# vituslcx/Shuffle-exchange

Hardware: AMD Instinct MI355X
Metric: tokens/sec Llama-3-8B ZeRO-3 bf16 (training, whole job) (higher is better)
Workload: dtype bf16; 1 GPU; llama8b-z3; model=llama3-8b, global_batch=16, seq_len=2048, micro_batch_per_gpu=8, grad_accum=2, parallelism=zero3-dp1, params=8030261248, activation_checkpointing=False, optimizer=AdamW(fp32 master, fused HIP), zero_knobs=tuned, sequence_parallel_size=1, expert_parallel_size=1

## Files before the change

csrc/kernels/gemm_wgrad.hip:

```cpp
#include "sxe_common.h"
#include <torch/library.h>

namespace sxe {
namespace wg {

constexpr int BM = 256, BN = 256, SLAB = 16;
constexpr int NWAVE = 8, NTHR = NWAVE * 64;
constexpr int ROWB = 256;
constexpr int HALF = SLAB * ROWB;
constexpr int SLOT = 4 * HALF;
constexpr int GROUP_M = 8;

typedef __bf16 bf16x8 __attribute__((ext_vector_type(8)));
typedef short i16x4 __attribute__((ext_vector_type(4)));
typedef short i16x8 __attribute__((ext_vector_type(8)));
typedef float f32x16 __attribute__((ext_vector_type(16)));

__device__ __forceinline__ int swz(int row) { return (row & 3) << 2; }

__device__ __forceinline__ i16x4 lds_tr(const char* base, int byte_off) {
  return __builtin_amdgcn_ds_read_tr16_b64_v4i16(
      (__attribute__((address_space(3))) i16x4*)(const_cast<char*>(base) + byte_off));
}

__device__ __forceinline__ int frag_off(int dt, int lane) {
  const int g = lane >> 4, i = lane & 15, q = i >> 2, p = i & 3, h = g >> 1;
  const int ch = 4 * dt + 2 * (g & 1) + (p >> 1);
  const int row = 4 * h + q;
  return row * ROWB + 16 * (ch ^ swz(row)) + 8 * (p & 1);
}

__device__ __forceinline__ bf16x8 frag_at(const char* lane_base, int row0) {
  i16x4 lo = lds_tr(lane_base, row0 * ROWB);
  i16x4 hi = lds_tr(lane_base, (row0 + 8) * ROWB);
  const i16x8 c = __builtin_shufflevector(lo, hi, 0, 1, 2, 3, 4, 5, 6, 7);
  return __builtin_bit_cast(bf16x8, c);
}

__device__ __forceinline__ void glds16(const void* gsrc, unsigned lds) {
  asm volatile("s_mov_b32 m0, %0\n\tglobal_load_lds_dwordx4 %1, off" ::"s"(lds), "v"(gsrc) : "memory", "m0");
}

struct DmaPlan {
  const unsigned short* a;
  const unsigned short* b;
  unsigned lds_a, lds_b;
};

__device__ __forceinline__ DmaPlan dma_plan(const unsigned short* A, int64_t lda, const unsigned short* B,
                                            int64_t ldb, int m0, int n0, unsigned lds_base) {
  const int lane = threadIdx.x & 63, w = threadIdx.x >> 6;
  const int half = (w >> 2) & 1, rq = w & 3;
  const int row = 4 * rq + (lane >> 4);
  const int ch = (lane & 15) ^ swz(row);
  DmaPlan d;
  d.a = A + (int64_t)row * lda + m0 + half * 128 + ch * 8;
  d.b = B + (int64_t)row * ldb + n0 + half * 128 + ch * 8;
  d.lds_a = __builtin_amdgcn_readfirstlane(lds_base + half * HALF + 4 * rq * ROWB);
  d.lds_b = __builtin_amdgcn_readfirstlane(lds_base + (2 + half) * HALF + 4 * rq * ROWB);
  return d;
}

__device__ __forceinline__ void load_slab(const DmaPlan& d, int64_t lda, int64_t ldb, int slab, int slot) {
  const int r = SLAB * slab;
  glds16(d.a + (int64_t)r * lda, d.lds_a + slot * SLOT);
  glds16(d.b + (int64_t)r * ldb, d.lds_b + slot * SLOT);
}

__device__ __forceinline__ int acc_row(int i, int h) { return (i & 3) + 8 * (i >> 2) + 4 * h; }

template <bool ACCUM, int R, bool STAGGER, bool NODMA = false, bool SEG2 = false>
__global__ void __launch_bounds__(NTHR, 1) wgrad_kernel(const unsigned short* __restrict__ A, int64_t lda,
                                                        const unsigned short* __restrict__ B, int64_t ldb,
                                                        float* __restrict__ C, int64_t ldc, int M, int N, int K,
                                                        float alpha, int group_m, const unsigned short* A2,
                                                        const unsigned short* B2, int ns1) {
  static_assert(R == 8, "fragment bases assume slots 0-3 / 4-7");
  constexpr int D = STAGGER ? R - 3 : R - 2;
  constexpr int WAIT = STAGGER ? 2 * (D - 2) : 2 * (D - 1);
  extern __shared__ __attribute__((aligned(1024))) char smem[];
  const int lane = threadIdx.x & 63, w = threadIdx.x >> 6;
  const int wr = w >> 2, wc = w & 3;
  const int tm = M / BM, tn = N / BN, nwg = tm * tn;
  const int orig = blockIdx.x;
  const int q = nwg / 8, r = nwg % 8, xcd = orig % 8;
  const int wgid = (xcd < r ? xcd * (q + 1) : r * (q + 1) + (xcd - r) * q) + orig / 8;
  const int per_group = group_m * tn;
  const int grp = wgid / per_group;
  const int first_m = grp * group_m;
  const int gsz = min(tm - first_m, group_m);
  const int bm = first_m + (wgid % per_group) % gsz;
  const int bn = (wgid % per_group) / gsz;
  const int m0 = bm * BM, n0 = bn * BN;

  f32x16 acc[4][2];
#pragma unroll
  for (int i = 0; i < 4; ++i)
#pragma unroll
    for (int j = 0; j < 2; ++j)
#pragma unroll
      for (int e = 0; e < 16; ++e) acc[i][j][e] = 0.f;

  const int ns = K / SLAB;
  bf16x8 fa[2][4], fb[2][2];
  const char* fbase[2][6];
#pragma unroll
  for (int h = 0; h < 2; ++h) {
#pragma unroll
    for (int i = 0; i < 4; ++i) fbase[h][i] = smem + 4 * h * SLOT + wr * HALF + frag_off(i, lane);
#pragma unroll
    for (int j = 0; j < 2; ++j)
      fbase[h][4 + j] = smem + 4 * h * SLOT + (2 + (wc >> 1)) * HALF + frag_off((wc & 1) * 2 + j, lane);
  }
  auto read_frags = [&](int slot, bf16x8 (&a)[4], bf16x8 (&b)[2]) {
#pragma unroll
    for (int i = 0; i < 4; ++i) a[i] = frag_at(fbase[slot >> 2][i] + (slot & 3) * SLOT, 0);
#pragma unroll
    for (int j = 0; j < 2; ++j) b[j] = frag_at(fbase[slot >> 2][4 + j] + (slot & 3) * SLOT, 0);
  };
  auto mma = [&](const bf16x8 (&a)[4], const bf16x8 (&b)[2]) {
    __builtin_amdgcn_s_setprio(1);
#pragma unroll
    for (int i = 0; i < 4; ++i)
#pragma unroll
      for (int j = 0; j < 2; ++j) acc[i][j] = __builtin_amdgcn_mfma_f32_32x32x16_bf16(a[i], b[j], acc[i][j], 0, 0, 0);
    __builtin_amdgcn_s_setprio(0);
  };
  const unsigned lds_base = (unsigned)(uintptr_t)(__attribute__((address_space(3))) char*)smem;
  const DmaPlan dp = dma_plan(A, lda, B, ldb, m0, n0, lds_base);
  const DmaPlan dp2 = SEG2 ? dma_plan(A2, lda, B2, ldb, m0, n0, lds_base) : dp;
  auto load_any = [&](int slab, int slot) {
    if (!SEG2 || slab < ns1)
      load_slab(dp, lda, ldb, slab, slot);
    else
      load_slab(dp2, lda, ldb, slab - ns1, slot);
  };
#pragma unroll
  for (int j = 0; j < D; ++j) load_any(j, j);
  asm volatile("s_waitcnt vmcnt(%0)" ::"n"(WAIT) : "memory");
  __builtin_amdgcn_s_barrier();
  read_frags(0, fa[0], fb[0]);
  if (STAGGER && __builtin_amdgcn_readfirstlane(wr) == 1) __builtin_amdgcn_s_barrier();
  for (int s0 = 0; s0 < ns; s0 += R) {
#pragma unroll
    for (int j = 0; j < R; ++j) {
      if (!NODMA) load_any(min(s0 + j + D, ns - 1), (j + D) % R);
      if (NODMA)
        asm volatile("s_waitcnt vmcnt(0)" ::: "memory");
      else
        asm volatile("s_waitcnt vmcnt(%0)" ::"n"(WAIT) : "memory");
      __builtin_amdgcn_s_barrier();
      read_frags((j + 1) % R, fa[(j + 1) & 1], fb[(j + 1) & 1]);
      mma(fa[j & 1], fb[j & 1]);
      if (STAGGER) __builtin_amdgcn_s_barrier();
    }
  }
  if (STAGGER && __builtin_amdgcn_readfirstlane(wr) == 0) __builtin_amdgcn_s_barrier();
  asm volatile("s_waitcnt vmcnt(0)" ::: "memory");
  const int h = lane >> 5, col = lane & 31;
#pragma unroll
  for (int i = 0; i < 4; ++i) {
    float* rowp[2];
    float old[2][16];
#pragma unroll
    for (int j = 0; j < 2; ++j) {
      rowp[j] = C + (int64_t)(m0 + wr * 128 + i * 32) * ldc + n0 + wc * 64 + j * 32 + col;
      if (ACCUM) {
#pragma unroll
        for (int e = 0; e < 16; ++e) old[j][e] = __builtin_nontemporal_load(rowp[j] + (int64_t)acc_row(e, h) * ldc);
      }
    }
#pragma unroll
    for (int j = 0; j < 2; ++j)
#pragma unroll
      for (int e = 0; e < 16; ++e) {
        const float v = alpha * acc[i][j][e];
        rowp[j][(int64_t)acc_row(e, h) * ldc] = ACCUM ? old[j][e] + v : v;
      }
  }
}


namespace w4 {
constexpr int SLAB = 32, R = 4, D = 3;
constexpr int NTHR = 256;
constexpr int HALF = SLAB * ROWB;
constexpr int SLOT = 4 * HALF;
constexpr int WAIT = 8 * (D - 1);

struct Plan {
  const unsigned short* a;
  const unsigned short* b;
  unsigned lds;
};

template <bool ACCUM>
__global__ void __launch_bounds__(NTHR, 1) kernel(const unsigned short* __restrict__ A, int64_t lda,
                                                  const unsigned short* __restrict__ B, int64_t ldb,
                                                  float* __restrict__ C, int64_t ldc, int M, int N, int K,
                                                  float alpha, int group_m, const unsigned short* A2,
                                                  const unsigned short* B2, int ns1) {
  extern __shared__ __attribute__((aligned(1024))) char smem[];
  const int lane = threadIdx.x & 63, w = threadIdx.x >> 6;
  const int wr = w >> 1, wc = w & 1;
  const int tm = M / BM, tn = N / BN, nwg = tm * tn;
  const int orig = blockIdx.x;
  const int q = nwg / 8, r = nwg % 8, xcd = orig % 8;
  const int wgid = (xcd < r ? xcd * (q + 1) : r * (q + 1) + (xcd - r) * q) + orig / 8;
  const int per_group = group_m * tn;
  const int grp = wgid / per_group;
  const int first_m = grp * group_m;
  const int gsz = min(tm - first_m, group_m);
  const int bm = first_m + (wgid % per_group) % gsz;
  const int bn = (wgid % per_group) / gsz;
  const int m0 = bm * BM, n0 = bn * BN;

  f32x16 acc[4][4];
#pragma unroll
  for (int i = 0; i < 4; ++i)
#pragma unroll
    for (int j = 0; j < 4; ++j)
#pragma unroll
      for (int e = 0; e < 16; ++e) acc[i][j][e] = 0.f;

  Plan pl, pl2;
  {
    const int row = lane >> 4;
    const int ch = (lane & 15) ^ swz(row);
    pl.a = A + (int64_t)row * lda + m0 + ch * 8;
    pl.b = B + (int64_t)row * ldb + n0 + ch * 8;
    pl.lds = (unsigned)(uintptr_t)(__attribute__((address_space(3))) char*)smem;
    pl2 = pl;
    pl2.a = A2 + (int64_t)row * lda + m0 + ch * 8;
    pl2.b = B2 + (int64_t)row * ldb + n0 + ch * 8;
  }
  const int ns1_32 = ns1 / 2;
  auto load_slab = [&](int slab_any, int slot) {
    const bool second = slab_any >= ns1_32;
    const Plan& P = second ? pl2 : pl;
    const int slab = second ? slab_any - ns1_32 : slab_any;
#pragma unroll
    for (int it = 0; it < 8; ++it) {
      const int op = it >> 2, half = (it >> 1) & 1, rq = (it & 1) * 4 + w;
      const int64_t rows = (int64_t)SLAB * slab + 4 * rq;
      const unsigned short* src = op == 0 ? P.a + rows * lda + half * 128 : P.b + rows * ldb + half * 128;
      const unsigned dst = __builtin_amdgcn_readfirstlane(pl.lds + slot * SLOT + (op * 2 + half) * HALF + 4 * rq * ROWB);
      glds16(src, dst);
    }
  };
  const char* fa_base[2][4];
  const char* fb_base[2][4];
#pragma unroll
  for (int hb = 0; hb < 2; ++hb)
#pragma unroll
    for (int i = 0; i < 4; ++i) {
      fa_base[hb][i] = smem + 2 * hb * SLOT + wr * HALF + frag_off(i, lane);
      fb_base[hb][i] = smem + 2 * hb * SLOT + (2 + wc) * HALF + frag_off(i, lane);
    }
  bf16x8 fa[2][2][4], fb[2][2][4];
  auto read_frags = [&](int slot, bf16x8 (&a)[2][4], bf16x8 (&b)[2][4]) {
#pragma unroll
    for (int kk = 0; kk < 2; ++kk)
#pragma unroll
      for (int i = 0; i < 4; ++i) {
        a[kk][i] = frag_at(fa_base[slot >> 1][i] + (slot & 1) * SLOT, 16 * kk);
        b[kk][i] = frag_at(fb_base[slot >> 1][i] + (slot & 1) * SLOT, 16 * kk);
      }
  };
  auto mma = [&](const bf16x8 (&a)[2][4], const bf16x8 (&b)[2][4]) {
    __builtin_amdgcn_s_setprio(1);
#pragma unroll
    for (int kk = 0; kk < 2; ++kk)
#pragma unroll
      for (int i = 0; i < 4; ++i)
#pragma unroll
        for (int j = 0; j < 4; ++j)
          acc[i][j] = __builtin_amdgcn_mfma_f32_32x32x16_bf16(a[kk][i], b[kk][j], acc[i][j], 0, 0, 0);
    __builtin_amdgcn_s_setprio(0);
  };
  const int ns = K / SLAB;
#pragma unroll
  for (int j = 0; j < D; ++j) load_slab(j, j);
  asm volatile("s_waitcnt vmcnt(%0)" ::"n"(WAIT) : "memory");
  __builtin_amdgcn_s_barrier();
  read_frags(0, fa[0], fb[0]);
  for (int s0 = 0; s0 < ns; s0 += R) {
#pragma unroll
    for (int j = 0; j < R; ++j) {
      load_slab(min(s0 + j + D, ns - 1), (j + D) % R);
      asm volatile("s_waitcnt vmcnt(%0)\n\ts_waitcnt lgkmcnt(0)" ::"n"(WAIT) : "memory");
      __builtin_amdgcn_s_barrier();
      read_frags((j + 1) % R, fa[(j + 1) & 1], fb[(j + 1) & 1]);
      mma(fa[j & 1], fb[j & 1]);
    }
  }
  asm volatile("s_waitcnt vmcnt(0)" ::: "memory");
  const int h = lane >> 5, col = lane & 31;
#pragma unroll
  for (int i = 0; i < 4; ++i) {
    float* rowp[4];
    float old[4][16];
#pragma unroll
    for (int j = 0; j < 4; ++j) {
      rowp[j] = C + (int64_t)(m0 + wr * 128 + i * 32) * ldc + n0 + wc * 128 + j * 32 + col;
      if (ACCUM) {
#pragma unroll
        for (int e = 0; e < 16; ++e) old[j][e] = __builtin_nontemporal_load(rowp[j] + (int64_t)acc_row(e, h) * ldc);
      }
    }
#pragma unroll
    for (int j = 0; j < 4; ++j)
#pragma unroll
      for (int e = 0; e < 16; ++e) {
        const float v = alpha * acc[i][j][e];
        rowp[j][(int64_t)acc_row(e, h) * ldc] = ACCUM ? old[j][e] + v : v;
      }
  }
}
}

}

bool wgrad_supported(const at::Tensor& a, const at::Tensor& b, const at::Tensor& c) {
  return a.is_cuda() && a.scalar_type() == at::kBFloat16 && b.scalar_type() == at::kBFloat16 &&
         c.scalar_type() == at::kFloat && a.dim() == 2 && b.dim() == 2 && c.dim() == 2 && a.stride(1) == 1 &&
         b.stride(1) == 1 && c.stride(1) == 1 && a.size(0) == b.size(0) && c.size(0) == a.size(1) &&
         c.size(1) == b.size(1) && a.size(1) % wg::BM == 0 && b.size(1) % wg::BN == 0 && a.size(0) % (8 * wg::SLAB) == 0 &&
         (reinterpret_cast<uintptr_t>(a.data_ptr()) % 16 == 0) && (reinterpret_cast<uintptr_t>(b.data_ptr()) % 16 == 0) &&
         a.stride(0) % 8 == 0 && b.stride(0) % 8 == 0;
}

static void wgrad_launch(const at::Tensor& a, const at::Tensor& b, const at::Tensor& a2, const at::Tensor& b2, int K,
                         int ns1, at::Tensor c, double alpha, bool accumulate, int64_t variant, bool seg2 = false) {
  c10::DeviceGuard g(a.device());
  const int M = a.size(1), N = b.size(1);
  const int nwg = (M / wg::BM) * (N / wg::BN);
  const size_t lds = 8 * wg::SLOT;
  using Kern = void (*)(const unsigned short*, int64_t, const unsigned short*, int64_t, float*, int64_t, int, int,
                        int, float, int, const unsigned short*, const unsigned short*, int);
  const int group_m = variant >= 16 ? (int)(variant >> 4) : wg::GROUP_M;
  variant &= 15;
  static const Kern kerns[5][2] = {{wg::wgrad_kernel<false, 8, false>, wg::wgrad_kernel<true, 8, false>},
                                   {wg::wgrad_kernel<false, 8, true>, wg::wgrad_kernel<true, 8, true>},
                                   {wg::w4::kernel<false>, wg::w4::kernel<true>},
                                   {wg::wgrad_kernel<false, 8, false, true>, wg::wgrad_kernel<true, 8, false, true>},
                                   {wg::wgrad_kernel<false, 8, false, false, true>,
                                    wg::wgrad_kernel<true, 8, false, false, true>}};
  static bool attr_set = [&] {
    for (auto& row : kerns)
      for (Kern k : row)
        SXE_HIP_CHECK(hipFuncSetAttribute((const void*)k, hipFuncAttributeMaxDynamicSharedMemorySize, (int)lds));
    return true;
  }();
  (void)attr_set;
  SXE_CHECK(variant >= 0 && variant <= 3, "wgrad_gemm_: variant must be 0..3");
  SXE_CHECK(!seg2 || variant == 0, "wgrad_gemm2_: the 8-wave lock-step schedule only");
  const int nthr = variant == 2 ? wg::w4::NTHR : wg::NTHR;
  hipLaunchKernelGGL(kerns[seg2 ? 4 : variant][accumulate ? 1 : 0], dim3(nwg), dim3(nthr), lds, cur_stream(),
                     reinterpret_cast<const unsigned short*>(a.data_ptr()), a.stride(0),
                     reinterpret_cast<const unsigned short*>(b.data_ptr()), b.stride(0), c.data_ptr<float>(),
                     c.stride(0), M, N, K, (float)alpha, group_m, reinterpret_cast<const unsigned short*>(a2.data_ptr()),
                     reinterpret_cast<const unsigned short*>(b2.data_ptr()), ns1);
  SXE_LAUNCH_CHECK();
}

void wgrad_gemm_variant_(const at::Tensor& a, const at::Tensor& b, at::Tensor c, double alpha, bool accumulate,
                         int64_t variant) {
  SXE_CHECK(wgrad_supported(a, b, c), "wgrad_gemm_: unsupported shapes/dtypes/strides");
  const int K = a.size(0);
  wgrad_launch(a, b, a, b, K, K / wg::SLAB, c, alpha, accumulate, variant);
}

static int64_t default_variant(const at::Tensor& a, const at::Tensor& b) {
  const int64_t tm = a.size(1) / wg::BM, tn = b.size(1) / wg::BN;
  return 0 + 16 * (tm >= 4 * tn ? 4 : 8);
}

void wgrad_gemm_(const at::Tensor& a, const at::Tensor& b, at::Tensor c, double alpha, bool accumulate) {
  wgrad_gemm_variant_(a, b, c, alpha, accumulate, default_variant(a, b));
}

bool wgrad2_supported(const at::Tensor& a, const at::Tensor& b, const at::Tensor& a2, const at::Tensor& b2,
                      const at::Tensor& c) {
  if (a2.dim() != 2 || b2.dim() != 2 || a2.scalar_type() != a.scalar_type() || b2.scalar_type() != b.scalar_type() ||
      a2.size(1) != a.size(1) || b2.size(1) != b.size(1) || a2.size(0) != b2.size(0) || a2.stride(1) != 1 ||
      b2.stride(1) != 1 || a2.stride(0) != a.stride(0) || b2.stride(0) != b.stride(0) || a.size(0) % 32 != 0 ||
      (reinterpret_cast<uintptr_t>(a2.data_ptr()) % 16) != 0 || (reinterpret_cast<uintptr_t>(b2.data_ptr()) % 16) != 0)
    return false;
  const int64_t K = a.size(0) + a2.size(0);
  if (K % (8 * wg::SLAB) != 0) return false;
  return a.is_cuda() && a.scalar_type() == at::kBFloat16 && b.scalar_type() == at::kBFloat16 &&
         c.scalar_type() == at::kFloat && a.dim() == 2 && b.dim() == 2 && c.dim() == 2 && a.stride(1) == 1 &&
         b.stride(1) == 1 && c.stride(1) == 1 && a.size(0) == b.size(0) && c.size(0) == a.size(1) &&
         c.size(1) == b.size(1) && a.size(1) % wg::BM == 0 && b.size(1) % wg::BN == 0 &&
         (reinterpret_cast<uintptr_t>(a.data_ptr()) % 16 == 0) && (reinterpret_cast<uintptr_t>(b.data_ptr()) % 16 == 0) &&
         a.stride(0) % 8 == 0 && b.stride(0) % 8 == 0;
}

void wgrad_gemm2_(const at::Tensor& a, const at::Tensor& b, const at::Tensor& a2, const at::Tensor& b2, at::Tensor c,
                  double alpha, bool accumulate) {
  SXE_CHECK(wgrad2_supported(a, b, a2, b2, c), "wgrad_gemm2_: unsupported shapes/dtypes/strides");
  const int K = (int)(a.size(0) + a2.size(0));
  wgrad_launch(a, b, a2, b2, K, (int)(a.size(0) / wg::SLAB), c, alpha, accumulate, default_variant(a, b), true);
}

}

TORCH_LIBRARY_FRAGMENT(sxe, m) {
  m.def("wgrad_gemm_(Tensor a, Tensor b, Tensor(a!) c, float alpha, bool accumulate) -> ()");
  m.def("wgrad_gemm_variant_(Tensor a, Tensor b, Tensor(a!) c, float alpha, bool accumulate, int variant) -> ()");
  m.def("wgrad_gemm2_(Tensor a, Tensor b, Tensor a2, Tensor b2, Tensor(a!) c, float alpha, bool accumulate) -> ()");
}
TORCH_LIBRARY_IMPL(sxe, CUDA, m) {
  m.impl("wgrad_gemm_", &sxe::wgrad_gemm_);
  m.impl("wgrad_gemm_variant_", &sxe::wgrad_gemm_variant_);
  m.impl("wgrad_gemm2_", &sxe::wgrad_gemm2_);
}
```

shuffle_exchange_amd/ops/linear.py:

```python
import os
import weakref

import torch
import torch.nn.functional as F

TN_MIN_ELEMS = int(os.environ.get("SXE_WGRAD_TN_MIN_ELEMS", 32 * 2**20))
TN_FP32_OUT = os.environ.get("SXE_WGRAD_TN_FP32OUT", "1") == "1"

SKINNY_MAX_M = int(os.environ.get("SXE_SKINNY_MAX_M", 4))


def _skinny(x, weight, bias):
    if torch.compiler.is_compiling():
        return None
    K = x.shape[-1]
    if not (x.is_cuda and x.dtype == torch.bfloat16 and weight.dtype == torch.bfloat16 and weight.dim() == 2
            and weight.is_contiguous() and K % 8 == 0 and weight.data_ptr() % 16 == 0):
        return None
    if bias is not None and not (bias.dtype == torch.bfloat16 and bias.is_contiguous()):
        return None
    x2 = x.reshape(-1, K)
    if not (0 < x2.shape[0] <= SKINNY_MAX_M and x2.stride(1) == 1 and x2.stride(0) % 8 == 0
            and x2.data_ptr() % 16 == 0):
        return None
    from . import native
    native.require_hip()
    return torch.ops.sxe.skinny_gemm(x2, weight, bias).view(*x.shape[:-1], weight.shape[0])


def _pro_weight(weight):
    if isinstance(weight, torch.Tensor):
        if weight.dtype == torch.bfloat16 and weight.dim() == 2 and weight.is_contiguous() and weight.data_ptr() % 16 == 0:
            return weight, None
        return None
    from .fp_quantizer import FP8Weight
    if not isinstance(weight, FP8Weight):
        return None
    q, sc = weight.q, weight.scale
    if q.element_size() == 1 and q.dim() == 2 and q.is_contiguous():
        return q.view(torch.uint8), sc
    return None


def _pro_ok(x, rows_max=4):
    return (x.is_cuda and x.dtype == torch.bfloat16 and x.dim() == 2 and 0 < x.shape[0] <= rows_max
            and x.stride(1) == 1 and x.stride(0) % 8 == 0 and x.data_ptr() % 16 == 0 and not x.requires_grad)


def fused_rms_linear(x, residual, norm_weight, eps, weight, bias=None):
    wk = _pro_weight(weight)
    if wk is None or not _pro_ok(x) or norm_weight.dtype != torch.bfloat16 or not norm_weight.is_contiguous():
        return None
    if residual is not None and (residual.shape != x.shape or residual.stride() != x.stride()
                                 or residual.dtype != x.dtype):
        return None
    w, sc = wk
    if x.shape[1] != w.shape[1]:
        return None
    y, h = torch.ops.sxe.skinny_gemm_pro(x, residual, norm_weight, float(eps), w, sc, bias, 1)
    return y, (h if residual is not None else x)


def fused_rms_rope_linear(x, residual, norm_weight, eps, weight, rope, positions, cache, slots, nq, nkv):
    wk = _pro_weight(weight)
    if (wk is None or not _pro_ok(x) or norm_weight.dtype != torch.bfloat16 or not norm_weight.is_contiguous()
            or rope.cos.shape[-1] != 64 or not cache.is_contiguous() or cache.dim() != 5 or cache.shape[-1] != 128):
        return None
    if residual is not None and (residual.shape != x.shape or residual.stride() != x.stride()
                                 or residual.dtype != x.dtype):
        return None
    w, sc = wk
    if x.shape[1] != w.shape[1] or w.shape[0] != (nq + 2 * nkv) * 128:
        return None
    y, h = torch.ops.sxe.skinny_gemm_pro_rope(x, residual, norm_weight, float(eps), w, sc, rope.cos, rope.sin,
                                              positions.reshape(-1).contiguous().long(), slots, cache, int(nq), int(nkv))
    return y, (h if residual is not None else x)


def fused_swiglu_linear(gu, weight, bias=None):
    wk = _pro_weight(weight)
    if wk is None or not _pro_ok(gu):
        return None
    w, sc = wk
    if gu.shape[1] != 2 * w.shape[1]:
        return None
    return torch.ops.sxe.skinny_gemm_pro(gu, None, None, 0.0, w, sc, bias, 2)[0]


def fused_merge_linear(part_o, part_ml, weight, bias=None):
    wk = _pro_weight(weight)
    if wk is None or not part_o.is_cuda or part_o.shape[1] > 4:
        return None
    w, sc = wk
    if w.shape[1] != part_o.shape[2] * part_o.shape[3]:
        return None
    return torch.ops.sxe.skinny_gemm_merge(part_o, part_ml, w, sc, bias)


SXE_WGRAD = os.environ.get("SXE_WGRAD", "1") == "1"
WGRAD_MIN_TILES = int(os.environ.get("SXE_WGRAD_MIN_TILES", "768"))


def _sxe_wgrad_ok(gy2, x2, buf):
    if not (SXE_WGRAD and gy2.is_cuda and buf.dtype == torch.float32 and gy2.dtype == torch.bfloat16
            and x2.dtype == torch.bfloat16 and buf.is_contiguous() and gy2.stride(1) == 1 and x2.stride(1) == 1):
        return False
    K, M, N = gy2.shape[0], gy2.shape[1], x2.shape[1]
    if K % 128 or M % 256 or N % 256 or gy2.stride(0) % 8 or x2.stride(0) % 8 or M * N >= 2 ** 27:
        return False
    tiles = (M // 256) * (N // 256)
    return tiles % 256 == 0 or tiles >= WGRAD_MIN_TILES


def _tn_ok(gy2, x2):
    return (gy2.is_cuda and gy2.dtype == torch.bfloat16 and x2.dtype == torch.bfloat16 and TN_MIN_ELEMS > 0
            and gy2.shape[1] * x2.shape[1] >= TN_MIN_ELEMS and gy2.shape[0] % 64 == 0 and gy2.shape[1] % 64 == 0
            and x2.shape[1] % 64 == 0 and gy2.is_contiguous() and x2.is_contiguous())


DGRAD_WT_MIN_ELEMS = int(os.environ.get("SXE_DGRAD_WT_MIN_ELEMS", 16 * 2**20))


WT_CACHE = False
WT_CACHE_MAX_BYTES = int(float(os.environ.get("SXE_WT_CACHE_GB", "20")) * 2**30)
_wt_cache = {}
_wt_cache_bytes = 0


def invalidate_transposed_weights():
    global _wt_cache_bytes
    _wt_cache.clear()
    _wt_cache_bytes = 0


def _transpose16(t):
    return torch.ops.sxe.transpose16(t)


def _transposed_weight(w):
    global _wt_cache_bytes
    if not WT_CACHE or not isinstance(w, torch.nn.Parameter):
        return _transpose16(w)
    hit = _wt_cache.get(id(w))
    if (hit is not None and hit[0]() is w and hit[1].shape == w.shape[::-1] and hit[2] == w.data_ptr()
            and hit[3] == w._version):
        return hit[1]
    if hit is not None:
        _wt_cache.pop(id(w))
        _wt_cache_bytes -= hit[1].numel() * hit[1].element_size()
    wt = _transpose16(w)
    nbytes = wt.numel() * wt.element_size()
    if _wt_cache_bytes + nbytes <= WT_CACHE_MAX_BYTES:
        _wt_cache[id(w)] = (weakref.ref(w), wt, w.data_ptr(), w._version)
        _wt_cache_bytes += nbytes
    return wt


def transposed_weight_cache_bytes():
    return _wt_cache_bytes


def configure_transposed_weight_cache(enabled, free_bytes=None):
    global WT_CACHE, WT_CACHE_MAX_BYTES
    WT_CACHE = bool(enabled)
    cap = int(float(os.environ.get("SXE_WT_CACHE_GB", "20")) * 2**30)
    if free_bytes is not None:
        cap = min(cap, int(free_bytes) // 4)
    WT_CACHE_MAX_BYTES = cap
    invalidate_transposed_weights()
    return cap


def data_grad(gy, w):
    if (DGRAD_WT_MIN_ELEMS > 0 and gy.is_cuda and gy.dtype == torch.bfloat16 and w.dtype == torch.bfloat16
            and w.dim() == 2 and w.is_contiguous() and w.numel() >= DGRAD_WT_MIN_ELEMS and w.shape[0] % 64 == 0
            and w.shape[1] % 64 == 0 and gy.numel() // gy.shape[-1] >= 2048):
        return torch.matmul(gy, _transposed_weight(w).t())
    return torch.matmul(gy, w)


def grad_target(w):
    tgt = getattr(w, "_sxe_grad_target", None)
    if tgt is None or getattr(w, "_sxe_grad_partial", False) or w.grad is not None:
        return None
    return tgt


def write_weight_grad(w, gy2, x2):
    tgt = grad_target(w)
    if tgt is None:
        return False
    buf, accumulate = tgt(w)
    if _sxe_wgrad_ok(gy2, x2, buf):
        torch.ops.sxe.wgrad_gemm_(gy2, x2, buf, 1.0, bool(accumulate))
    elif _tn_ok(gy2, x2) and buf.is_contiguous():
        a, b = torch.ops.sxe.transpose16(gy2), torch.ops.sxe.transpose16(x2).t()
        if buf.dtype == gy2.dtype and not accumulate:
            torch.mm(a, b, out=buf)
        elif buf.dtype == torch.float32 and TN_FP32_OUT:
            torch.ops.aten.addmm.dtype_out(buf, a, b, torch.float32, beta=1 if accumulate else 0, alpha=1, out=buf)
        else:
            dw = torch.mm(a, b).view_as(buf)
            buf.add_(dw) if accumulate else buf.copy_(dw)
    elif buf.dtype == torch.float32 and gy2.dtype != torch.float32:
        if gy2.is_cuda:
            torch.ops.aten.addmm.dtype_out(buf, gy2.t(), x2, torch.float32, beta=1 if accumulate else 0, alpha=1,
                                           out=buf)
        else:
            dw = (gy2.t() @ x2).float()
            buf.add_(dw) if accumulate else buf.copy_(dw)
    elif accumulate:
        buf.addmm_(gy2.t(), x2)
    else:
        torch.mm(gy2.t(), x2, out=buf)
    w._sxe_grad_done(w)
    return True


def _autocast_dtype(x):
    dev = x.device.type
    if dev in ("cuda", "cpu") and torch.is_autocast_enabled(dev):
        return torch.get_autocast_dtype(dev)
    return None


class _Linear(torch.autograd.Function):
    @staticmethod
    def forward(ctx, x, weight, bias):
        ctx.param = None
        ac = _autocast_dtype(x)
        if ac is not None and weight.dtype != ac:
            ctx.param = weight
            x, weight = x.to(ac), weight.to(ac)
            bias = bias.to(ac) if bias is not None else None
        ctx.save_for_backward(x, weight)
        ctx.has_bias = bias is not None
        return F.linear(x, weight, bias)

    @staticmethod
    def backward(ctx, gy):
        x, w = ctx.saved_tensors
        wp = ctx.param if ctx.param is not None else w
        if gy.dtype != x.dtype:
            gy = gy.to(x.dtype)
        gy2 = gy.reshape(-1, gy.shape[-1])
        dx = dw = db = None
        if ctx.needs_input_grad[0]:
            dx = data_grad(gy, w)
        if ctx.needs_input_grad[1]:
            x2 = x.reshape(-1, x.shape[-1])
            if not write_weight_grad(wp, gy2, x2):
                dw = gy2.t() @ x2
        if ctx.has_bias and ctx.needs_input_grad[2]:
            db = gy2.sum(0)
        return dx, dw, db


def linear(x, weight, bias=None):
    if not isinstance(weight, torch.Tensor):
        return weight.linear(x, bias)
    grad = torch.is_grad_enabled() and (weight.requires_grad or x.requires_grad)
    if grad and weight.requires_grad and hasattr(weight, "_sxe_grad_target"):
        return _Linear.apply(x, weight, bias)
    if not grad and SKINNY_MAX_M > 0 and x.is_cuda:
        y = _skinny(x, weight, bias)
        if y is not None:
            return y
    return F.linear(x, weight, bias)


class Linear(torch.nn.Linear):

    _sxe_lower_precision_safe = True

    def __init__(self, in_features, out_features, bias=True, device=None, dtype=None, init_std=None):
        super().__init__(in_features, out_features, bias=bias, device=device, dtype=dtype)
        if init_std is not None:
            with torch.no_grad():
                self.weight.normal_(0.0, init_std)
                if self.bias is not None:
                    self.bias.zero_()
            self._sxe_inited = True

    def forward(self, x, skip_bias=False):
        return linear(x, self.weight, None if skip_bias else self.bias)


class Embedding(torch.nn.Embedding):

    def __init__(self, num_embeddings, embedding_dim, init_std=None, **kw):
        super().__init__(num_embeddings, embedding_dim, **kw)
        if init_std is not None:
            with torch.no_grad():
                self.weight.normal_(0.0, init_std)
            self._sxe_inited = True
```

Measured before the change: 25850 tokens/s.

## Add 4-wave deep-pipelined wgrad GEMM kernel and make it the default

```diff
diff --git a/csrc/kernels/gemm_wgrad.hip b/csrc/kernels/gemm_wgrad.hip
--- a/csrc/kernels/gemm_wgrad.hip
+++ b/csrc/kernels/gemm_wgrad.hip
@@ -1,5 +1,6 @@
 #include "sxe_common.h"
 #include <torch/library.h>
+#include <cstdlib>
 
 namespace sxe {
 namespace wg {
@@ -319,6 +320,125 @@
 }
 }
 
+namespace w4p {
+using w4::HALF;
+using w4::NTHR;
+using w4::SLAB;
+using w4::SLOT;
+constexpr int R = 4, D = 4;
+constexpr int WAIT = 8 * (D - 2);
+
+template <bool ACCUM>
+__global__ void __launch_bounds__(NTHR, 1) kernel(const unsigned short* __restrict__ A, int64_t lda,
+                                                  const unsigned short* __restrict__ B, int64_t ldb,
+                                                  float* __restrict__ C, int64_t ldc, int M, int N, int K,
+                                                  float alpha, int group_m, const unsigned short* A2,
+                                                  const unsigned short* B2, int ns1) {
+  extern __shared__ __attribute__((aligned(1024))) char smem[];
+  const int lane = threadIdx.x & 63, w = threadIdx.x >> 6;
+  const int wr = w >> 1, wc = w & 1;
+  const int tm = M / BM, tn = N / BN, nwg = tm * tn;
+  const int orig = blockIdx.x;
+  const int q = nwg / 8, r = nwg % 8, xcd = orig % 8;
+  const int wgid = (xcd < r ? xcd * (q + 1) : r * (q + 1) + (xcd - r) * q) + orig / 8;
+  const int per_group = group_m * tn;
+  const int grp = wgid / per_group;
+  const int first_m = grp * group_m;
+  const int gsz = min(tm - first_m, group_m);
+  const int bm = first_m + (wgid % per_group) % gsz;
+  const int bn = (wgid % per_group) / gsz;
+  const int m0 = bm * BM, n0 = bn * BN;
+
+  f32x16 acc[4][4];
+#pragma unroll
+  for (int i = 0; i < 4; ++i)
+#pragma unroll
+    for (int j = 0; j < 4; ++j)
+#pragma unroll
+      for (int e = 0; e < 16; ++e) acc[i][j][e] = 0.f;
+
+  const int drow = lane >> 4;
+  const int dch = (lane & 15) ^ swz(drow);
+  const unsigned short* pa = A + (int64_t)drow * lda + m0 + dch * 8;
+  const unsigned short* pb = B + (int64_t)drow * ldb + n0 + dch * 8;
+  const unsigned lds0 = (unsigned)(uintptr_t)(__attribute__((address_space(3))) char*)smem;
+  auto dma = [&](int it, int slab, int slot) {
+    const int op = it >> 2, half = (it >> 1) & 1, rq = (it & 1) * 4 + w;
+    const int64_t rows = (int64_t)SLAB * slab + 4 * rq;
+    const unsigned short* src = op == 0 ? pa + rows * lda + half * 128 : pb + rows * ldb + half * 128;
+    glds16(src, __builtin_amdgcn_readfirstlane(lds0 + slot * SLOT + (op * 2 + half) * HALF + 4 * rq * ROWB));
+  };
+  const char* fa_base[2][4];
+  const char* fb_base[2][4];
+#pragma unroll
+  for (int hb = 0; hb < 2; ++hb)
+#pragma unroll
+    for (int i = 0; i < 4; ++i) {
+      fa_base[hb][i] = smem + 2 * hb * SLOT + wr * HALF + frag_off(i, lane);
+      fb_base[hb][i] = smem + 2 * hb * SLOT + (2 + wc) * HALF + frag_off(i, lane);
+    }
+  bf16x8 fa[2][2][4], fb[2][2][4];
+  auto read_frag = [&](int slot, int f, bf16x8 (&a)[2][4], bf16x8 (&b)[2][4]) {
+    const int kk = f >> 3, i = f & 3;
+    if ((f & 4) == 0)
+      b[kk][i] = frag_at(fb_base[slot >> 1][i] + (slot & 1) * SLOT, 16 * kk);
+    else
+      a[kk][i] = frag_at(fa_base[slot >> 1][i] + (slot & 1) * SLOT, 16 * kk);
+  };
+  const int ns = K / SLAB;
+#pragma unroll
+  for (int j = 0; j < D; ++j)
+#pragma unroll
+    for (int it = 0; it < 8; ++it) dma(it, j, j);
+  asm volatile("s_waitcnt vmcnt(%0)" ::"n"(8 * (D - 1)) : "memory");
+  __builtin_amdgcn_s_barrier();
+#pragma unroll
+  for (int f = 0; f < 16; ++f) read_frag(0, f, fa[0], fb[0]);
+  for (int s0 = 0; s0 < ns; s0 += R) {
+#pragma unroll
+    for (int j = 0; j < R; ++j) {
+      asm volatile("s_waitcnt vmcnt(%0)\n\ts_waitcnt lgkmcnt(0)" ::"n"(WAIT) : "memory");
+      __builtin_amdgcn_s_barrier();
+      __builtin_amdgcn_sched_barrier(0);
+      const int nslab = min(s0 + j + D, ns - 1);
+#pragma unroll
+      for (int g = 0; g < 8; ++g) {
+        const int kk = g >> 2, i = g & 3;
+        dma(g, nslab, j);
+        read_frag((j + 1) % R, 2 * g, fa[(j + 1) & 1], fb[(j + 1) & 1]);
+        read_frag((j + 1) % R, 2 * g + 1, fa[(j + 1) & 1], fb[(j + 1) & 1]);
+#pragma unroll
+        for (int jj = 0; jj < 4; ++jj)
+          acc[i][jj] = __builtin_amdgcn_mfma_f32_32x32x16_bf16(fa[j & 1][kk][i], fb[j & 1][kk][jj], acc[i][jj], 0, 0, 0);
+        __builtin_amdgcn_sched_barrier(0);
+      }
+    }
+  }
+  asm volatile("s_waitcnt vmcnt(0)" ::: "memory");
+  const int h = lane >> 5, col = lane & 31;
+#pragma unroll
+  for (int i = 0; i < 4; ++i) {
+    float* rowp[4];
+    float old[4][16];
+#pragma unroll
+    for (int j = 0; j < 4; ++j) {
+      rowp[j] = C + (int64_t)(m0 + wr * 128 + i * 32) * ldc + n0 + wc * 128 + j * 32 + col;
+      if (ACCUM) {
+#pragma unroll
+        for (int e = 0; e < 16; ++e) old[j][e] = __builtin_nontemporal_load(rowp[j] + (int64_t)acc_row(e, h) * ldc);
+      }
+    }
+#pragma unroll
+    for (int j = 0; j < 4; ++j)
+#pragma unroll
+      for (int e = 0; e < 16; ++e) {
+        const float v = alpha * acc[i][j][e];
+        rowp[j][(int64_t)acc_row(e, h) * ldc] = ACCUM ? old[j][e] + v : v;
+      }
+  }
+}
+}
+
 }
 
 bool wgrad_supported(const at::Tensor& a, const at::Tensor& b, const at::Tensor& c) {
@@ -340,10 +460,11 @@
                         int, float, int, const unsigned short*, const unsigned short*, int);
   const int group_m = variant >= 16 ? (int)(variant >> 4) : wg::GROUP_M;
   variant &= 15;
-  static const Kern kerns[5][2] = {{wg::wgrad_kernel<false, 8, false>, wg::wgrad_kernel<true, 8, false>},
+  static const Kern kerns[6][2] = {{wg::wgrad_kernel<false, 8, false>, wg::wgrad_kernel<true, 8, false>},
                                    {wg::wgrad_kernel<false, 8, true>, wg::wgrad_kernel<true, 8, true>},
                                    {wg::w4::kernel<false>, wg::w4::kernel<true>},
                                    {wg::wgrad_kernel<false, 8, false, true>, wg::wgrad_kernel<true, 8, false, true>},
+                                   {wg::w4p::kernel<false>, wg::w4p::kernel<true>},
                                    {wg::wgrad_kernel<false, 8, false, false, true>,
                                     wg::wgrad_kernel<true, 8, false, false, true>}};
   static bool attr_set = [&] {
@@ -353,10 +474,10 @@
     return true;
   }();
   (void)attr_set;
-  SXE_CHECK(variant >= 0 && variant <= 3, "wgrad_gemm_: variant must be 0..3");
+  SXE_CHECK(variant >= 0 && variant <= 4, "wgrad_gemm_: variant must be 0..4");
   SXE_CHECK(!seg2 || variant == 0, "wgrad_gemm2_: the 8-wave lock-step schedule only");
-  const int nthr = variant == 2 ? wg::w4::NTHR : wg::NTHR;
-  hipLaunchKernelGGL(kerns[seg2 ? 4 : variant][accumulate ? 1 : 0], dim3(nwg), dim3(nthr), lds, cur_stream(),
+  const int nthr = variant == 2 || variant == 4 ? wg::w4::NTHR : wg::NTHR;
+  hipLaunchKernelGGL(kerns[seg2 ? 5 : variant][accumulate ? 1 : 0], dim3(nwg), dim3(nthr), lds, cur_stream(),
                      reinterpret_cast<const unsigned short*>(a.data_ptr()), a.stride(0),
                      reinterpret_cast<const unsigned short*>(b.data_ptr()), b.stride(0), c.data_ptr<float>(),
                      c.stride(0), M, N, K, (float)alpha, group_m, reinterpret_cast<const unsigned short*>(a2.data_ptr()),
@@ -371,9 +492,18 @@
   wgrad_launch(a, b, a, b, K, K / wg::SLAB, c, alpha, accumulate, variant);
 }
 
+static int64_t default_group_m(const at::Tensor& a, const at::Tensor& b) {
+  const int64_t tm = a.size(1) / wg::BM, tn = b.size(1) / wg::BN;
+  return tm >= 4 * tn ? 4 : 8;
+}
+
+constexpr int64_t DEFAULT_SCHEDULE = 4;
 static int64_t default_variant(const at::Tensor& a, const at::Tensor& b) {
-  const int64_t tm = a.size(1) / wg::BM, tn = b.size(1) / wg::BN;
-  return 0 + 16 * (tm >= 4 * tn ? 4 : 8);
+  static const int64_t forced = [] {
+    const char* e = std::getenv("SXE_WGRAD_VARIANT");
+    return e && *e >= '0' && *e <= '4' && !e[1] ? (int64_t)(*e - '0') : (int64_t)-1;
+  }();
+  return (forced >= 0 ? forced : DEFAULT_SCHEDULE) + 16 * default_group_m(a, b);
 }
 
 void wgrad_gemm_(const at::Tensor& a, const at::Tensor& b, at::Tensor c, double alpha, bool accumulate) {
@@ -401,7 +531,7 @@
                   double alpha, bool accumulate) {
   SXE_CHECK(wgrad2_supported(a, b, a2, b2, c), "wgrad_gemm2_: unsupported shapes/dtypes/strides");
   const int K = (int)(a.size(0) + a2.size(0));
-  wgrad_launch(a, b, a2, b2, K, (int)(a.size(0) / wg::SLAB), c, alpha, accumulate, default_variant(a, b), true);
+  wgrad_launch(a, b, a2, b2, K, (int)(a.size(0) / wg::SLAB), c, alpha, accumulate, 0 + 16 * default_group_m(a, b), true);
 }
 
 }
diff --git a/shuffle_exchange_amd/ops/linear.py b/shuffle_exchange_amd/ops/linear.py
--- a/shuffle_exchange_amd/ops/linear.py
+++ b/shuffle_exchange_amd/ops/linear.py
@@ -97,7 +97,7 @@
     return torch.ops.sxe.skinny_gemm_merge(part_o, part_ml, w, sc, bias)
 
 
-SXE_WGRAD = os.environ.get("SXE_WGRAD", "1") == "1"
+SXE_WGRAD =os.environ.get("SXE_WGRAD", "1") == "1"
 WGRAD_MIN_TILES = int(os.environ.get("SXE_WGRAD_MIN_TILES", "768"))
 
 
```

Result: no change. 25890 tokens/s (median of 2 runs) (+0.1%).
